# bupt-cist/vqa-playground-pytorch

Measured on AMD Instinct MI355X. Metric: VQA samples/sec (fwd+bwd), CoR2 batch 512, 36x2048 regions, higher is better.
Workload: dtype f32

## Files before the change

### vqa_playground_pytorch_amd/csrc/bilinear_rt.hip

```cpp
#include <cstdlib>

#include "bilinear_folded.hpp"
#include "gemm_f32_rt.hpp"

namespace vqa {
namespace {

struct FoldRtArgs {
  const float* x;
  const float* w[2];
  const float* bias[2];
  const float* h2;
  float* out;
  int ldx, ldw, ldh2, ldo;
  int B, N, K, NO;
  int tiles_o;
};

constexpr int kNB = 3;

template <bool FWD, int S, int IB, int R, int FG = 1>
__global__ __launch_bounds__(rt::kThreads, 1) void bilinear_fold_rt_kernel(FoldRtArgs p) {
  using rt::f32x4;
  const int lane = threadIdx.x & 63, r = lane & 15, g = lane >> 4;
  const int wave = __builtin_amdgcn_readfirstlane(threadIdx.x >> 6);
  const int tile = xcd_remap(blockIdx.x, gridDim.x);
  const int b0 = (tile / p.tiles_o) * S;
  const int o0 = (tile % p.tiles_o) * (64 * IB) + wave * (16 * IB);
  const int B = p.B, N = p.N, K = p.K, NO = p.NO;
  if (o0 >= NO) return;

  rt::rsrc_t Wb[R];
#pragma unroll
  for (int rk = 0; rk < R; ++rk) Wb[rk] = rt::make_rsrc(p.w[rk], ((size_t)(NO - 1) * p.ldw + K) * 4);
  const rt::rsrc_t Xb = rt::make_rsrc(p.x, ((size_t)(B * N - 1) * p.ldx + K) * 4);
  const rt::rsrc_t Hb = rt::make_rsrc(p.h2, (size_t)B * R * p.ldh2 * 4);
  uint32_t offW[IB], offX[S][kNB], offH[S];
#pragma unroll
  for (int i = 0; i < IB; ++i) offW[i] = ((uint32_t)min(o0 + 16 * i + r, NO - 1) * (uint32_t)p.ldw + 4u * g) * 4u;
#pragma unroll
  for (int s = 0; s < S; ++s) {
    const int b = min(b0 + s, B - 1);
#pragma unroll
    for (int j = 0; j < kNB; ++j) offX[s][j] = ((uint32_t)(b * N + min(16 * j + r, N - 1)) * (uint32_t)p.ldx + 4u * g) * 4u;
    offH[s] = (uint32_t)(b * R) * (uint32_t)p.ldh2 * 4u;
  }
  float hrow[FWD ? S : 1][R][FWD ? IB : 1];
  if constexpr (FWD) {
#pragma unroll
    for (int s = 0; s < S; ++s)
#pragma unroll
      for (int rk = 0; rk < R; ++rk)
#pragma unroll
        for (int i = 0; i < IB; ++i)
          hrow[s][rk][i] = rt::ldg4(Hb, offH[s] + (uint32_t)(rk * p.ldh2 + min(o0 + 16 * i + r, NO - 1)) * 4u, 0u);
  }

  f32x4 acc[S][IB][kNB];
#pragma unroll
  for (int s = 0; s < S; ++s)
#pragma unroll
    for (int i = 0; i < IB; ++i)
#pragma unroll
      for (int j = 0; j < kNB; ++j) acc[s][i][j] = f32x4{0.f, 0.f, 0.f, 0.f};

  struct Frag {
    f32x4 w[R][IB];
    f32x4 x[S][kNB];
    f32x4 hk[FWD ? 1 : S][R];
  };
  auto load = [&](Frag& f, int c) {
    const uint32_t so = (uint32_t)c * 64u;
#pragma unroll
    for (int rk = 0; rk < R; ++rk)
#pragma unroll
      for (int i = 0; i < IB; ++i) f.w[rk][i] = rt::ldg16(Wb[rk], offW[i], so);
#pragma unroll
    for (int s = 0; s < S; ++s) {
#pragma unroll
      for (int j = 0; j < kNB; ++j) f.x[s][j] = rt::ldg16(Xb, offX[s][j], so);
      if constexpr (!FWD) {
#pragma unroll
        for (int rk = 0; rk < R; ++rk) f.hk[s][rk] = rt::ldg16(Hb, offH[s] + (uint32_t)(rk * p.ldh2) * 4u + 16u * g, so);
      }
    }
  };
  auto fold = [&](const Frag& f, int s, int i) -> f32x4 {
    typedef float f32x2 __attribute__((ext_vector_type(2)));
    f32x4 we;
    if constexpr (FWD) {
      const f32x2 h0 = f32x2{hrow[s][0][i], hrow[s][0][i]};
      f32x2 lo = f32x2{f.w[0][i][0], f.w[0][i][1]} * h0, hi = f32x2{f.w[0][i][2], f.w[0][i][3]} * h0;
      if constexpr (R == 2) {
        const f32x2 h1 = f32x2{hrow[s][1][i], hrow[s][1][i]};
        lo = __builtin_elementwise_fma(f32x2{f.w[1][i][0], f.w[1][i][1]}, h1, lo);
        hi = __builtin_elementwise_fma(f32x2{f.w[1][i][2], f.w[1][i][3]}, h1, hi);
      }
      we = f32x4{lo[0], lo[1], hi[0], hi[1]};
    } else {
      f32x2 lo = f32x2{f.w[0][i][0], f.w[0][i][1]} * f32x2{f.hk[s][0][0], f.hk[s][0][1]};
      f32x2 hi = f32x2{f.w[0][i][2], f.w[0][i][3]} * f32x2{f.hk[s][0][2], f.hk[s][0][3]};
      if constexpr (R == 2) {
        lo = __builtin_elementwise_fma(f32x2{f.w[1][i][0], f.w[1][i][1]}, f32x2{f.hk[s][1][0], f.hk[s][1][1]}, lo);
        hi = __builtin_elementwise_fma(f32x2{f.w[1][i][2], f.w[1][i][3]}, f32x2{f.hk[s][1][2], f.hk[s][1][3]}, hi);
      }
      we = f32x4{lo[0], lo[1], hi[0], hi[1]};
    }
    return we;
  };
  auto compute = [&](const Frag& f, auto pin, auto nloads) {
    constexpr bool PIN = decltype(pin)::value;
    constexpr int NL = decltype(nloads)::value;
    constexpr int NQ = S * IB;
    constexpr int NV = R == 2 ? 4 : 2;
    f32x4 we[FG], wn[FG];
#pragma unroll
    for (int t = 0; t < FG; ++t) we[t] = fold(f, min(t, NQ - 1) / IB, min(t, NQ - 1) % IB);
    if constexpr (PIN) __builtin_amdgcn_sched_group_barrier(0x002, NV * FG, 0);
    int issued = 0;
#pragma unroll
    for (int q0 = 0; q0 < NQ; q0 += FG) {
#pragma unroll
      for (int t = 0; t < FG; ++t) wn[t] = we[t];
      if (q0 + FG < NQ) {
#pragma unroll
        for (int t = 0; t < FG; ++t)
          if (q0 + FG + t < NQ) {
            wn[t] = fold(f, (q0 + FG + t) / IB, (q0 + FG + t) % IB);
            if constexpr (PIN) __builtin_amdgcn_sched_group_barrier(0x002, NV, 0);
          }
      }
#pragma unroll
      for (int t = 0; t < FG; ++t) {
        const int q = q0 + t;
        if (q >= NQ) break;
        const int s = q / IB, i = q % IB;
#pragma unroll
        for (int kb = 0; kb < 4; ++kb)
#pragma unroll
          for (int j = 0; j < kNB; ++j) {
            acc[s][i][j] = __builtin_amdgcn_mfma_f32_16x16x4f32(we[t][kb], f.x[s][j][kb], acc[s][i][j], 0, 0, 0);
            if constexpr (PIN) {
              __builtin_amdgcn_sched_group_barrier(0x008, 1, 0);
              const int m = q * 4 * kNB + kb * kNB + j;
              if (issued < NL && (m + 1) * NL / (NQ * 4 * kNB) > issued) {
                __builtin_amdgcn_sched_group_barrier(0x020, 1, 0);
                ++issued;
              }
            }
          }
      }
#pragma unroll
      for (int t = 0; t < FG; ++t) we[t] = wn[t];
    }
  };
  auto step = [&](Frag& fn, int cn, const Frag& f) {
    constexpr int NL = R * IB + S * kNB + (FWD ? 0 : S * R);
    load(fn, cn);
    compute(f, std::true_type{}, std::integral_constant<int, NL>{});
    __builtin_amdgcn_sched_barrier(0);
  };

  const int nfull = K >> 4;
  const int c_pairs = nfull & ~1;
  {
    Frag f0, f1;
    if (c_pairs > 0) {
      load(f0, 0);
      __builtin_amdgcn_sched_barrier(0);
      for (int c = 0; c < c_pairs; c += 2) {
        step(f1, c + 1, f0);
        step(f0, min(c + 2, c_pairs - 1), f1);
      }
    }
    if (c_pairs < nfull) {
      load(f0, c_pairs);
      compute(f0, std::false_type{}, std::integral_constant<int, 0>{});
    }
  }
  if ((K & 15) != 0 || FWD) {
    Frag f;
#pragma unroll
    for (int kb = 0; kb < 4; ++kb) {
      const int k = 16 * nfull + 4 * g + kb;
      const bool in = k < K;
      const uint32_t kc = (uint32_t)min(k, K - 1);
#pragma unroll
      for (int rk = 0; rk < R; ++rk)
#pragma unroll
        for (int i = 0; i < IB; ++i) {
          float v = rt::ldg4(Wb[rk], offW[i] - 16u * g + kc * 4u, 0u);
          v = in ? v : 0.f;
          if constexpr (FWD) {
            if (k == K) v = p.bias[rk][min(o0 + 16 * i + r, NO - 1)];
          }
          f.w[rk][i][kb] = v;
        }
#pragma unroll
      for (int s = 0; s < S; ++s) {
#pragma unroll
        for (int j = 0; j < kNB; ++j) {
          float v = rt::ldg4(Xb, offX[s][j] - 16u * g + kc * 4u, 0u);
          v = in ? v : 0.f;
          if constexpr (FWD) {
            if (k == K) v = 1.f;
          }
          f.x[s][j][kb] = v;
        }
        if constexpr (!FWD) {
#pragma unroll
          for (int rk = 0; rk < R; ++rk) {
            const float v = rt::ldg4(Hb, offH[s] + (uint32_t)(rk * p.ldh2) * 4u + kc * 4u, 0u);
            f.hk[s][rk][kb] = in ? v : 0.f;
          }
        }
      }
    }
    compute(f, std::false_type{}, std::integral_constant<int, 0>{});
  }

#pragma unroll
  for (int s = 0; s < S; ++s) {
    const int b = b0 + s;
    if (b >= B) break;
#pragma unroll
    for (int j = 0; j < kNB; ++j) {
      const int n = 16 * j + r;
      if (n >= N) continue;
      float* __restrict__ row = p.out + (size_t)(b * N + n) * p.ldo;
#pragma unroll
      for (int i = 0; i < IB; ++i) {
        const int o = o0 + 16 * i + 4 * g;
        if (o + 3 < NO) {
          *reinterpret_cast<f32x4*>(row + o) = acc[s][i][j];
        } else {
#pragma unroll
          for (int t = 0; t < 4; ++t)
            if (o + t < NO) row[o + t] = acc[s][i][j][t];
        }
      }
    }
  }
}

template <bool FWD>
int launch(const FoldRtArgs& a0, int R, hipStream_t s) {
  FoldRtArgs a = a0;
  constexpr int S = FWD ? 4 : 2, IB = FWD ? 4 : 5;
  a.tiles_o = (a.NO + 64 * IB - 1) / (64 * IB);
  const dim3 grid((unsigned)(((a.B + S - 1) / S) * a.tiles_o));
  const char* fg_opt = vqa::option("VQA_K4_FG");
  const int fg = fg_opt != nullptr ? std::atoi(fg_opt) : (FWD ? 4 : 2);
  if (R == 1)
    VQA_LAUNCH((bilinear_fold_rt_kernel<FWD, S, IB, 1>), grid, dim3(rt::kThreads), 0, s, a);
  else if (fg == 2)
    VQA_LAUNCH((bilinear_fold_rt_kernel<FWD, S, IB, 2, 2>), grid, dim3(rt::kThreads), 0, s, a);
  else if (fg == 4)
    VQA_LAUNCH((bilinear_fold_rt_kernel<FWD, S, IB, 2, 4>), grid, dim3(rt::kThreads), 0, s, a);
  else
    VQA_LAUNCH((bilinear_fold_rt_kernel<FWD, S, IB, 2>), grid, dim3(rt::kThreads), 0, s, a);
  return check_launch(FWD ? "lowrank_bilinear_fusion_folded_fwd (register-tile)" : "lowrank_bilinear_fusion_folded_bwd (dx, register-tile)");
}

}

bool fold_rt_supported(int B, int N, int K, int NO, int R, int ldx, int ldw, int ldo) {
  const bool off = vqa::option_is("VQA_K4_RT", '0');
  return !off && R >= 1 && R <= 2 && N > 16 && N <= 48 && B >= 256 && K >= 32 && NO >= 64 && ldx % 2 == 0 && ldw % 2 == 0 &&
         ldo % 2 == 0 && (size_t)B * N * (size_t)(ldx > ldo ? ldx : ldo) * 4 < (1ull << 32) && (size_t)NO * ldw * 4 < (1ull << 32);
}

int fold_rt_forward(const float* x, int ldx, const float* const* w1, const float* const* b1, const float* h2, float* out, int B,
                    int N, int L, int H, int R, hipStream_t s) {
  FoldRtArgs a{};
  a.x = x;
  for (int r = 0; r < R; ++r) {
    a.w[r] = w1[r];
    a.bias[r] = b1[r];
  }
  a.h2 = h2;
  a.out = out;
  a.ldx = ldx;
  a.ldw = L;
  a.ldh2 = H;
  a.ldo = H;
  a.B = B;
  a.N = N;
  a.K = L;
  a.NO = H;
  return launch<true>(a, R, s);
}

int fold_rt_data_gradient(const float* g, const float* const* w1t, const float* h2, float* d_x, int B, int N, int L, int H, int R,
                          hipStream_t s) {
  FoldRtArgs a{};
  a.x = g;
  for (int r = 0; r < R; ++r) a.w[r] = w1t[r];
  a.h2 = h2;
  a.out = d_x;
  a.ldx = H;
  a.ldw = H;
  a.ldh2 = H;
  a.ldo = L;
  a.B = B;
  a.N = N;
  a.K = H;
  a.NO = L;
  return launch<false>(a, R, s);
}

}
```

Before: 262,000.

## Share one MFMA block across four samples for the 4-region tail in folded bilinear forward

With N=36 regions, the forward kernel used three 16-row region blocks per sample, so the third block was mostly padding (4 of 16 rows). The new tail path covers only two full blocks per sample. The remaining 4 regions of all four samples are packed into one shared 16-row block that multiplies the unfolded low-rank weights, and the h2 factors are applied afterward in the epilogue. This cuts wasted MFMA work and X loads, at the cost of extra accumulators (R*IB), extra h2 loads in the epilogue, and a kernel with two template bodies behind a runtime branch.

```diff
diff --git a/vqa_playground_pytorch_amd/csrc/bilinear_rt.hip b/vqa_playground_pytorch_amd/csrc/bilinear_rt.hip
--- a/vqa_playground_pytorch_amd/csrc/bilinear_rt.hip
+++ b/vqa_playground_pytorch_amd/csrc/bilinear_rt.hip
@@ -15,13 +15,18 @@
   int ldx, ldw, ldh2, ldo;
   int B, N, K, NO;
   int tiles_o;
+  int tail;
 };
 
 constexpr int kNB = 3;
 
-template <bool FWD, int S, int IB, int R, int FG = 1>
-__global__ __launch_bounds__(rt::kThreads, 1) void bilinear_fold_rt_kernel(FoldRtArgs p) {
+template <bool FWD, int S, int IB, int R, int FG, bool TAIL>
+__device__ __forceinline__ void fold_rt_body(const FoldRtArgs& p) {
   using rt::f32x4;
+  typedef float f32x2 __attribute__((ext_vector_type(2)));
+  static_assert(!TAIL || (FWD && S == 4), "the shared tail block: four samples of four regions, fold factors along the rows");
+  constexpr int NBF = TAIL ? 2 : kNB;
+  constexpr int NT = TAIL ? 1 : 0;
   const int lane = threadIdx.x & 63, r = lane & 15, g = lane >> 4;
   const int wave = __builtin_amdgcn_readfirstlane(threadIdx.x >> 6);
   const int tile = xcd_remap(blockIdx.x, gridDim.x);
@@ -35,16 +40,18 @@
   for (int rk = 0; rk < R; ++rk) Wb[rk] = rt::make_rsrc(p.w[rk], ((size_t)(NO - 1) * p.ldw + K) * 4);
   const rt::rsrc_t Xb = rt::make_rsrc(p.x, ((size_t)(B * N - 1) * p.ldx + K) * 4);
   const rt::rsrc_t Hb = rt::make_rsrc(p.h2, (size_t)B * R * p.ldh2 * 4);
-  uint32_t offW[IB], offX[S][kNB], offH[S];
+  uint32_t offW[IB], offX[S][NBF], offH[S];
 #pragma unroll
   for (int i = 0; i < IB; ++i) offW[i] = ((uint32_t)min(o0 + 16 * i + r, NO - 1) * (uint32_t)p.ldw + 4u * g) * 4u;
 #pragma unroll
   for (int s = 0; s < S; ++s) {
     const int b = min(b0 + s, B - 1);
 #pragma unroll
-    for (int j = 0; j < kNB; ++j) offX[s][j] = ((uint32_t)(b * N + min(16 * j + r, N - 1)) * (uint32_t)p.ldx + 4u * g) * 4u;
+    for (int j = 0; j < NBF; ++j) offX[s][j] = ((uint32_t)(b * N + min(16 * j + r, N - 1)) * (uint32_t)p.ldx + 4u * g) * 4u;
     offH[s] = (uint32_t)(b * R) * (uint32_t)p.ldh2 * 4u;
   }
+  const int bt = min(b0 + (r >> 2), B - 1);
+  const uint32_t offT = ((uint32_t)(bt * N + min(32 + (r & 3), N - 1)) * (uint32_t)p.ldx + 4u * g) * 4u;
   float hrow[FWD ? S : 1][R][FWD ? IB : 1];
   if constexpr (FWD) {
 #pragma unroll
@@ -56,17 +63,25 @@
           hrow[s][rk][i] = rt::ldg4(Hb, offH[s] + (uint32_t)(rk * p.ldh2 + min(o0 + 16 * i + r, NO - 1)) * 4u, 0u);
   }
 
-  f32x4 acc[S][IB][kNB];
+  f32x4 acc[S][IB][NBF];
 #pragma unroll
   for (int s = 0; s < S; ++s)
 #pragma unroll
     for (int i = 0; i < IB; ++i)
 #pragma unroll
-      for (int j = 0; j < kNB; ++j) acc[s][i][j] = f32x4{0.f, 0.f, 0.f, 0.f};
+      for (int j = 0; j < NBF; ++j) acc[s][i][j] = f32x4{0.f, 0.f, 0.f, 0.f};
+  f32x4 accT[TAIL ? R : 1][TAIL ? IB : 1];
+  if constexpr (TAIL) {
+#pragma unroll
+    for (int rk = 0; rk < R; ++rk)
+#pragma unroll
+      for (int i = 0; i < IB; ++i) accT[rk][i] = f32x4{0.f, 0.f, 0.f, 0.f};
+  }
 
   struct Frag {
     f32x4 w[R][IB];
-    f32x4 x[S][kNB];
+    f32x4 x[S][NBF];
+    f32x4 xt;
     f32x4 hk[FWD ? 1 : S][R];
   };
   auto load = [&](Frag& f, int c) {
@@ -78,15 +93,15 @@
 #pragma unroll
     for (int s = 0; s < S; ++s) {
 #pragma unroll
-      for (int j = 0; j < kNB; ++j) f.x[s][j] = rt::ldg16(Xb, offX[s][j], so);
+      for (int j = 0; j < NBF; ++j) f.x[s][j] = rt::ldg16(Xb, offX[s][j], so);
       if constexpr (!FWD) {
 #pragma unroll
         for (int rk = 0; rk < R; ++rk) f.hk[s][rk] = rt::ldg16(Hb, offH[s] + (uint32_t)(rk * p.ldh2) * 4u + 16u * g, so);
       }
     }
+    if constexpr (TAIL) f.xt = rt::ldg16(Xb, offT, so);
   };
   auto fold = [&](const Frag& f, int s, int i) -> f32x4 {
-    typedef float f32x2 __attribute__((ext_vector_type(2)));
     f32x4 we;
     if constexpr (FWD) {
       const f32x2 h0 = f32x2{hrow[s][0][i], hrow[s][0][i]};
@@ -117,7 +132,29 @@
 #pragma unroll
     for (int t = 0; t < FG; ++t) we[t] = fold(f, min(t, NQ - 1) / IB, min(t, NQ - 1) % IB);
     if constexpr (PIN) __builtin_amdgcn_sched_group_barrier(0x002, NV * FG, 0);
+    constexpr int NMT = NT * R * IB * 4;
+    constexpr int NM = NMT + NQ * 4 * NBF;
     int issued = 0;
+    auto pin_mfma = [&](int m) {
+      if constexpr (PIN) {
+        __builtin_amdgcn_sched_group_barrier(0x008, 1, 0);
+        if (issued < NL && (m + 1) * NL / NM > issued) {
+          __builtin_amdgcn_sched_group_barrier(0x020, 1, 0);
+          ++issued;
+        }
+      }
+    };
+    if constexpr (TAIL) {
+#pragma unroll
+      for (int kb = 0; kb < 4; ++kb)
+#pragma unroll
+        for (int rk = 0; rk < R; ++rk)
+#pragma unroll
+          for (int i = 0; i < IB; ++i) {
+            accT[rk][i] = __builtin_amdgcn_mfma_f32_16x16x4f32(f.w[rk][i][kb], f.xt[kb], accT[rk][i], 0, 0, 0);
+            pin_mfma((kb * R + rk) * IB + i);
+          }
+    }
 #pragma unroll
     for (int q0 = 0; q0 < NQ; q0 += FG) {
 #pragma unroll
@@ -138,16 +175,9 @@
 #pragma unroll
         for (int kb = 0; kb < 4; ++kb)
 #pragma unroll
-          for (int j = 0; j < kNB; ++j) {
+          for (int j = 0; j < NBF; ++j) {
             acc[s][i][j] = __builtin_amdgcn_mfma_f32_16x16x4f32(we[t][kb], f.x[s][j][kb], acc[s][i][j], 0, 0, 0);
-            if constexpr (PIN) {
-              __builtin_amdgcn_sched_group_barrier(0x008, 1, 0);
-              const int m = q * 4 * kNB + kb * kNB + j;
-              if (issued < NL && (m + 1) * NL / (NQ * 4 * kNB) > issued) {
-                __builtin_amdgcn_sched_group_barrier(0x020, 1, 0);
-                ++issued;
-              }
-            }
+            pin_mfma(NMT + q * 4 * NBF + kb * NBF + j);
           }
       }
 #pragma unroll
@@ -155,7 +185,7 @@
     }
   };
   auto step = [&](Frag& fn, int cn, const Frag& f) {
-    constexpr int NL = R * IB + S * kNB + (FWD ? 0 : S * R);
+    constexpr int NL = R * IB + S * NBF + NT + (FWD ? 0 : S * R);
     load(fn, cn);
     compute(f, std::true_type{}, std::integral_constant<int, NL>{});
     __builtin_amdgcn_sched_barrier(0);
@@ -199,7 +229,7 @@
 #pragma unroll
       for (int s = 0; s < S; ++s) {
 #pragma unroll
-        for (int j = 0; j < kNB; ++j) {
+        for (int j = 0; j < NBF; ++j) {
           float v = rt::ldg4(Xb, offX[s][j] - 16u * g + kc * 4u, 0u);
           v = in ? v : 0.f;
           if constexpr (FWD) {
@@ -215,6 +245,12 @@
           }
         }
       }
+      if constexpr (TAIL) {
+        float v = rt::ldg4(Xb, offT - 16u * g + kc * 4u, 0u);
+        v = in ? v : 0.f;
+        if (k == K) v = 1.f;
+        f.xt[kb] = v;
+      }
     }
     compute(f, std::false_type{}, std::integral_constant<int, 0>{});
   }
@@ -224,7 +260,7 @@
     const int b = b0 + s;
     if (b >= B) break;
 #pragma unroll
-    for (int j = 0; j < kNB; ++j) {
+    for (int j = 0; j < NBF; ++j) {
       const int n = 16 * j + r;
       if (n >= N) continue;
       float* __restrict__ row = p.out + (size_t)(b * N + n) * p.ldo;
@@ -241,6 +277,56 @@
       }
     }
   }
+  if constexpr (TAIL) {
+    const int b = b0 + (r >> 2), n = 32 + (r & 3);
+    if (b < B && n < N) {
+      float* __restrict__ row = p.out + (size_t)(b * N + n) * p.ldo;
+#pragma unroll
+      for (int i = 0; i < IB; ++i) {
+        const int o = o0 + 16 * i + 4 * g;
+        if (o >= NO) continue;
+        const bool whole = o + 3 < NO;
+        f32x2 lo, hi;
+#pragma unroll
+        for (int rk = 0; rk < R; ++rk) {
+          const uint32_t oh = ((uint32_t)(b * R + rk) * (uint32_t)p.ldh2 + (uint32_t)o) * 4u;
+          f32x4 h;
+          if (whole) {
+            h = rt::ldg16(Hb, oh, 0u);
+          } else {
+#pragma unroll
+            for (int t = 0; t < 4; ++t) h[t] = rt::ldg4(Hb, oh - (uint32_t)o * 4u + (uint32_t)min(o + t, NO - 1) * 4u, 0u);
+          }
+          if (rk == 0) {
+            lo = f32x2{accT[0][i][0], accT[0][i][1]} * f32x2{h[0], h[1]};
+            hi = f32x2{accT[0][i][2], accT[0][i][3]} * f32x2{h[2], h[3]};
+          } else {
+            lo = __builtin_elementwise_fma(f32x2{accT[rk][i][0], accT[rk][i][1]}, f32x2{h[0], h[1]}, lo);
+            hi = __builtin_elementwise_fma(f32x2{accT[rk][i][2], accT[rk][i][3]}, f32x2{h[2], h[3]}, hi);
+          }
+        }
+        const f32x4 v = f32x4{lo[0], lo[1], hi[0], hi[1]};
+        if (whole) {
+          *reinterpret_cast<f32x4*>(row + o) = v;
+        } else {
+#pragma unroll
+          for (int t = 0; t < 4; ++t)
+            if (o + t < NO) row[o + t] = v[t];
+        }
+      }
+    }
+  }
+}
+
+template <bool FWD, int S, int IB, int R, int FG = 1>
+__global__ __launch_bounds__(rt::kThreads, 1) void bilinear_fold_rt_kernel(FoldRtArgs p) {
+  if constexpr (FWD && S == 4) {
+    if (p.tail != 0 && 32 < p.N && p.N <= 36) {
+      fold_rt_body<FWD, S, IB, R, FG, true>(p);
+      return;
+    }
+  }
+  fold_rt_body<FWD, S, IB, R, FG, false>(p);
 }
 
 template <bool FWD>
@@ -251,6 +337,7 @@
   const dim3 grid((unsigned)(((a.B + S - 1) / S) * a.tiles_o));
   const char* fg_opt = vqa::option("VQA_K4_FG");
   const int fg = fg_opt != nullptr ? std::atoi(fg_opt) : (FWD ? 4 : 2);
+  a.tail = FWD && !vqa::option_is("VQA_K4_TAIL", '0') ? 1 : 0;
   if (R == 1)
     VQA_LAUNCH((bilinear_fold_rt_kernel<FWD, S, IB, 1>), grid, dim3(rt::kThreads), 0, s, a);
   else if (fg == 2)
```

Result: no change. 263,800, median of 6 (+0.7%).
